# andvg3/LipVQ-VAE

Measured on AMD Instinct MI355X. Metric: actions tokenized/sec (encode+quantize) at B=4096 T=128 K=1024, 1/2/4/8 GPU, higher is better.
Workload: dtype f32

## Files before the change

lipvq-vae_amd/_capi.py:

```python
from __future__ import annotations

import ctypes as C
from pathlib import Path

import torch

import os as _os

_LIB_PATH = Path(_os.environ.get("LIPVQ_HIP_LIBRARY") or (Path(__file__).resolve().parent / "_lipvq_hip.so"))

ACT_NONE, ACT_GELU, ACT_SIGMOID, ACT_RELU = 0, 1, 2, 3
DIST_NORM, DIST_SQSUM = 0, 1
ABI_VERSION = 1

_vp, _i, _i64, _sz = C.c_void_p, C.c_int, C.c_int64, C.c_size_t

SIGNATURES = {
    "lipvq_abi_version": (_i, []),
    "lipvq_last_error": (C.c_char_p, []),
    "lipvq_set_option": (_i, [C.c_char_p, C.c_char_p]),
    "lipvq_get_option": (C.c_char_p, [C.c_char_p]),
    "lipvq_lipschitz_scale_f32": (_i, [_vp, _vp, _vp, _vp, _i, _i, _vp]),
    "lipvq_mlp3_packed_floats": (_sz, [_i, _i, _i, _i]),
    "lipvq_mlp3_pack_f32": (_i, [_vp] * 7 + [_i] * 4 + [_vp]),
# ... 115 lines not shown
            "(python -c 'import __graft_entry__ as g; g.build()' or make -C lipvq-vae_amd/csrc). "
            "There is no CPU fallback for the tokenizer path.")
    lib = C.CDLL(str(_LIB_PATH))
    for name, (res, args) in SIGNATURES.items():
        fn = getattr(lib, name)
        fn.restype, fn.argtypes = res, args
    got = lib.lipvq_abi_version()
    if got != ABI_VERSION:
        raise ImportError(f"lipvq ABI version {got} != expected {ABI_VERSION}")
    return lib


lib = _load()


OPTIONS = ("screen_mode", "tok_shape", "tok_ze_rows", "tok_inplace", "tok_defer_ze", "tok_nt_ze")


def set_option(name: str, value=None) -> None:
    v = None if value is None else str(value).encode()
    if lib.lipvq_set_option(name.encode(), v) != 0:
        raise LipvqLibraryError(lib.lipvq_last_error().decode(errors="replace"))


def get_option(name: str):
    v = lib.lipvq_get_option(name.encode())
    return None if v is None else v.decode()


if _os.environ.get("LIPVQ_DEV_KNOBS") == "1":
    for _o in OPTIONS:
# ... 10 lines not shown
```

lipvq-vae_amd/csrc/lipvq_fused.hip:

```cpp
#include <string.h>
#include <atomic>

#include "lipvq_mlp.h"
#include "lipvq_screen.h"
#include "lipvq_fused_lds.h"

#define FUSED_WAVES 8
#define FUSED_THREADS (FUSED_WAVES * 64)

struct Gelu2 {
    lq_v2f x, t, u, s;
    __device__ __forceinline__ void stage0(float a, float b) {
        x = (lq_v2f){a, b};
        t = x * x;
        u = lq_fma2(t, lq_bc2(0.11111111111111111111f), lq_bc2(-1.0f));
        s = lq_fma2(lq_bc2(0.00012666420661844313f), u, lq_bc2(-0.00043783686123788357f));
        s = lq_fma2(s, u, lq_bc2(0.0008924771682359278f));
    }
    __device__ __forceinline__ void stage1() {
        s = lq_fma2(s, u, lq_bc2(-0.002175821689888835f));
        s = lq_fma2(s, u, lq_bc2(0.005515238270163536f));
        s = lq_fma2(s, u, lq_bc2(-0.01217574905604124f));
        s = lq_fma2(s, u, lq_bc2(0.02415713667869568f));
    }
// ... 47 lines not shown
    int A, D, K;
    float gamma;
    int coarse;
    int inplace;
    int defer_ze;
    int nt_ze;
    int ze_ring;
    int keepz;
};

#ifdef LQ_STAMPS
#define LQ_STAMPS_ENTER()                                                                                            \
    const long long st_top = __builtin_amdgcn_s_memtime();                                                           \
    const long long st_top_rt = (long long)__builtin_amdgcn_s_memrealtime()
#define LQ_STAMPS_PROLOGUE_DONE()                                                                                    \
    long long st_acc[8] = {0, 0, 0, 0, 0, 0, 0, 0}, st_prev;                                                         \
    const long long st_begin = __builtin_amdgcn_s_memtime()
#define LQ_STAMPS_BEGIN_BLOCK() st_prev = __builtin_amdgcn_s_memtime()
#define LQ_STAMP(i) do { const long long t_ = __builtin_amdgcn_s_memtime(); st_acc[i] += t_ - st_prev; st_prev = t_; } while (0)
#define LQ_STAMPS_FLUSH(a, lane, wave, WAVES)                                                                        \
    if (lane == 0) {                                                                                                 \
        long long* dbg = LqWorkspace::from_lists(a.amb_list, a.N).stamps() + ((size_t)blockIdx.x * WAVES + wave) * 16;   \
        for (int i = 0; i < 7; ++i) dbg[i] = st_acc[i];                                                              \
        dbg[7] = 0;                                                                                                  \
        dbg[8] = __builtin_amdgcn_s_memtime() - st_begin;                                                            \
        dbg[9] = st_begin;                                                                                           \
        dbg[10] = st_begin - st_top;                                                                                 \
        dbg[11] = (long long)__builtin_amdgcn_s_memrealtime();                                                       \
        dbg[12] = st_top_rt;                                                                                         \
    }
#else
#define LQ_STAMPS_ENTER() do { } while (0)
#define LQ_STAMPS_PROLOGUE_DONE() do { } while (0)
#define LQ_STAMPS_BEGIN_BLOCK() do { } while (0)
#define LQ_STAMP(i) do { } while (0)
#define LQ_STAMPS_FLUSH(a, lane, wave, WAVES) do { } while (0)
#endif

template <int S, bool TRAIN>
__device__ __forceinline__ void tok_store_ze_tile(const TokArgs& a, const int h, const int64_t ze_shift, const int64_t row, const int t,
                                                  const f32x16& acc) {
    float lo8[8], hi8[8];
#pragma unroll
    for (int j = 0; j < 8; ++j) {
        const auto sw = __builtin_amdgcn_permlane32_swap(__float_as_uint(acc[j]), __float_as_uint(acc[8 + j]), false, false);
        lo8[j] = __uint_as_float(sw[0]);
        hi8[j] = __uint_as_float(sw[1]);
    }
    if (row < a.N && 2 * t + h < S) {
        float4* dst = reinterpret_cast<float4*>(a.ze_out + (size_t)(row - ze_shift) * a.D + 32 * t + 16 * h);
// ... 179 lines not shown
    const unsigned char* src = reinterpret_cast<const unsigned char*>(a.w2q) + (size_t)t_ * (G2 * 1024);
    unsigned char* dst = stage0 + (size_t)buf_ * SLAB_STRIDE;
    unsigned lane16 = (unsigned)lane * 16u;
    asm volatile("" : "+v"(lane16));
#pragma unroll
    for (int j = 0; j < G2 * 1024 / 1024 / WAVES; ++j) {
        const int off = (wave + j * WAVES) * 1024;
        const unsigned long long gaddr = (unsigned long long)(uintptr_t)(src + off) + lane16;
        const unsigned ldsaddr = __builtin_amdgcn_readfirstlane((unsigned)(uintptr_t)(dst + off));
        unsigned m0_keep;
        asm volatile("s_mov_b32 %0, m0\n\ts_mov_b32 m0, %2\n\ts_nop 0\n\tglobal_load_lds_dwordx4 %1, off\n\ts_mov_b32 m0, %0"
                     : "=&s"(m0_keep) : "v"(gaddr), "s"(ldsaddr) : "memory");
    }
}

template <int S, bool FAST, bool TRAIN, int WAVES, bool COARSE = false, bool VQ = false, bool KEEPZ = false>
__device__ __forceinline__ void tokenize_body(const TokArgs& a) {
    static_assert(!(FAST && TRAIN), "training uses the parity arithmetic");
    static_assert(!VQ || !FAST, "the ReLU instance: parity arithmetic");
    static_assert(!KEEPZ || (S <= 4 && !FAST && !TRAIN && !COARSE && !VQ), "z_e kept in registers: the narrow parity instances, decided in place");
    constexpr int THREADS = WAVES * 64;
    constexpr int TCF = COARSE ? fused_ring_tc_coarse(S) : fused_ring_tc(S), NBF = fused_ring_nb(S);
    using Lds = FusedLds<S, FAST>;
    static_assert(Lds::template slices_fit<WAVES, COARSE, KEEPZ>(), "the per-wave slices of the stage ring");
    constexpr size_t SLAB_STRIDE = Lds::SLAB_STRIDE;
    constexpr int T0 = Lds::T0, T1 = Lds::T1, T2 = Lds::T2;
    constexpr int S1 = Lds::S1, S2 = Lds::S2;
    constexpr bool STREAM2 = Lds::STREAM2;
    static_assert(!FAST || (S % 2 == 0 && S <= 8), "fast mode: D in {32, 64, 128}");
    extern __shared__ __attribute__((aligned(16))) unsigned char lds[];
    LQ_STAMPS_ENTER();

    const PackedLayout PL = packed_layout(a.A, 32 * T0, 32 * T1, 16 * S);
    const PrepLayout L = prep_layout(a.K, a.D);
    const int S0 = PL.S0;
    const int S0q = (S0 + 3) / 4;
    const int S0h = (a.A + 15) / 16;
    const Lds lay(a.A);
    float* const w_P0 = reinterpret_cast<float*>(lds);
    float* const w_B0 = w_P0 + lay.template n_P0<int>();
    float* const w_P1 = w_B0 + Lds::N_B0;
    float* const w_B1 = w_P1 + Lds::N_P1;
    float* const w_P2 = w_B1 + Lds::N_B1;
    float* const w_B2 = w_P2 + Lds::N_P2;
    float* const w_mu = w_B2 + Lds::N_B2;
    unsigned char* const stage0 = reinterpret_cast<unsigned char*>(w_mu + Lds::N_MU);
    unsigned* const hist = reinterpret_cast<unsigned*>(stage0 + Lds::template hist_in_ring<COARSE>());
    constexpr size_t STAGES_BYTES = Lds::template stages_bytes<COARSE>(), WSLICE = Lds::template wslice<WAVES, COARSE>();
    const bool use_hist = a.usage && Lds::hist_fits(a.A, a.K);

    const int tid = threadIdx.x, lane = tid & 63;
    const int wave = __builtin_amdgcn_readfirstlane(tid >> 6);
    const int ln = lane & 31, h = lane >> 5;

    const unsigned* hdr = reinterpret_cast<const unsigned*>(a.prep);
    const unsigned char* tiles = a.prep + (COARSE ? L.o_tiles_hi : L.o_tiles);
    const size_t tile_bytes = COARSE ? L.tile_bytes_hi : L.tile_bytes;
    const int sz = lq_scale_exp(1.0f + __uint_as_float(hdr[4]));
    const float fz = lq_pow2f(sz);
    const float fown = lq_pow2f(sz + (int)hdr[3]);
    const float tiny2 = (float)(16 * S) * lq_pow2f(-10 - 2 * sz);
    const int64_t nblk = (a.N + WAVES * 32 - 1) / (WAVES * 32);
    constexpr int XPF = 8;
// ... 156 lines not shown
                }
                if constexpr (KEEPZ) {
                    zkeep[t] = acc;
                } else if (a.ze_out) {
                    if (DEFER_ZE && a.defer_ze && t == T2 - 1) zdef = acc;
                    else store_ze_tile(row, t, acc);
                }
            };

            if constexpr (!FAST) {
                auto bias16 = [&](const float* wb, int t) { return tok_bias16(wb, t, h); };
                f32x16 h0[T0];
                constexpr int NTRIP = (16 * S + 63) / 64;
                constexpr int GP = (STAGES_BYTES >= (size_t)WAVES * 8192) ? 8 : 4;
                constexpr int NROUND = NTRIP * (8 / GP);
                unsigned char* gstage = stage0 + (size_t)wave * WSLICE;
                const bool gnow = DEFER_GATHER && have_pend && a.zq;
                if (gnow) lq_gather_dma<GP>(gstage, a.cb, pend_k, pend_ok, pend_row0, a.N, a.D, lane, 0, 0);
                {
#pragma unroll
                    for (int t = 0; t < T0; ++t) h0[t] = bias16(w_B0, t);
                    if (x_pref) {
#pragma unroll
                        for (int sq = 0; sq < XPF / 4; ++sq) {
                            if (sq < S0q) {
                                float4 av[T0];
#pragma unroll
                                for (int t = 0; t < T0; ++t) av[t] = *reinterpret_cast<const float4*>(w_P0 + ((t * S0q + sq) * 64 + lane_w) * 4);
#pragma unroll
                                for (int q = 0; q < 4; ++q) {
                                    const float bv = tok_x_masked<X_BATCHED, XPF>(x_kmax, 4 * sq + q, xq);
#pragma unroll
                                    for (int t = 0; t < T0; ++t) {
// ... 32 lines not shown
#pragma unroll
                            for (int r = 0; r < 16; ++r) h0[t][r] = pre[r] > 0.0f ? pre[r] : 0.0f;
                        } else if constexpr (LOCKSTEP) {
                            tok_gelu_poly_tile(h0[t], pre);
                            tok_gelu_fixup_lumped(h0[t], pre);
                        } else {
#pragma unroll
                            for (int r = 0; r < 16; r += 2) {
                                const lq_v2f g2 = lq_gelu_poly2((lq_v2f){pre[r], pre[r + 1]});
                                h0[t][r] = g2.x; h0[t][r + 1] = g2.y;
                            }
                            tok_gelu_fixup(h0[t], pre);
                        }
                    }
                }
                if (gnow) {
#pragma unroll
                    for (int rd = 0; rd < NROUND; ++rd) {
                        lq_wait_vmcnt<0>();
                        lq_gather_flush<GP>(gstage, a.zq, pend_ok, pend_row0, a.N, a.D, lane, rd / (8 / GP), GP * (rd % (8 / GP)));
                        if (rd + 1 < NROUND) {
                            asm volatile("s_waitcnt lgkmcnt(0)" ::: "memory");
                            lq_gather_dma<GP>(gstage, a.cb, pend_k, pend_ok, pend_row0, a.N, a.D, lane, (rd + 1) / (8 / GP),
                                              GP * ((rd + 1) % (8 / GP)));
                        }
                    }
                }
                LQ_STAMP(0);
                f32x16 h1[T1];
                f32x16 pend;
                constexpr int G1 = S1 / 4, G2 = S2 / 4;
// ... 140 lines not shown
        for (int r = 0; r < 16; ++r) { m1[r] = INFINITY; m2[r] = INFINITY; k1[r] = 0; }
        LQ_STAMP(3);
        constexpr bool DEFER_X = S <= 4 && !FAST && !TRAIN && !COARSE && !VQ;
        const int64_t blk_next = blk + gridDim.x < nblk ? blk + gridDim.x : blk;
        if (!DEFER_X && x_pref) load_x(blk_next, xq);
        constexpr bool PACKF = S <= 4 || S > 8 || COARSE;
        const float zn = COARSE ? lq_coarse_zn(row_a2, row_n2, row_fz, row_fown, __uint_as_float(hdr[5])) : 0.0f;
        float znr[16];
        if constexpr (COARSE) lq_row_factors(zn, lane, znr);
        else {
#pragma unroll
            for (int r = 0; r < 16; ++r) znr[r] = 0.0f;
        }
        if constexpr (KEEPZ) {
            auto deferred_x = [&]() { load_x(blk_next, xq); };
            lq_screen_core<S, THREADS, TCF, NBF, PACKF, COARSE, 0, decltype(deferred_x), DEFER_X ? XPF : 0>(
                ah, al, tiles, L.ntiles, stage0, tid, frow, znr, m1, m2, k1, false, deferred_x, true, DEFER_X && x_pref);
        } else {
            const bool have_def = DEFER_ZE && a.defer_ze && a.ze_out != nullptr;
            const bool wave_def = __builtin_amdgcn_ballot_w64(row < a.N) != 0ull;
            auto deferred_ze = [&]() {
                if (have_def) store_ze_tile(row, T2 - 1, zdef);
                if (DEFER_X && x_pref) load_x(blk_next, xq);
            };
            lq_screen_core<S, THREADS, TCF, NBF, PACKF, COARSE, 4, decltype(deferred_ze), DEFER_X ? XPF : 0>(
                ah, al, tiles, L.ntiles, stage0, tid, frow, znr, m1, m2, k1, have_def, deferred_ze, wave_def, DEFER_X && x_pref);
        }
        LQ_STAMP(4);
        const unsigned keep_mask = PACKF ? ~((1u << lq_pack_bits(L.ntiles)) - 1u) : 0xffffffffu;
        unsigned char* scratch = stage0 + (size_t)wave * WSLICE;
        int my_k;
        LqDecision dec;
        bool certified = lq_screen_decide<PACKF, COARSE>(m1, m2, k1, scratch, hdr, row_n2, row_fown, a.gamma, a.K, a.D, lane,
                                                         my_k, dec, PACKF ? lq_pow2f(lq_pack_bits(L.ntiles) - 23) : 0.0f, keep_mask,
                                                         zn, tiles, tile_bytes, ScreenCfg<S, TCF, COARSE>::FRAG_BYTES);
        const bool row_sane = VQ || row_n2 >= tiny2;
        certified = certified && row_sane;
        if constexpr (KEEPZ)
            certified = lq_screen_decide_inplace<PACKF, 2 * S, LIPVQ_DIST_NORM, T2>(
                dec, certified, row_sane, my_k, row0, row < a.N, a.amb_count, nullptr, a.cb, a.K, lane, keep_mask, scratch, zkeep);
        else if (!COARSE && a.inplace)
            certified = lq_screen_decide_inplace<PACKF, 2 * S, VQ ? LIPVQ_DIST_SQSUM : LIPVQ_DIST_NORM>(
                dec, certified, row_sane, my_k, row0 - ze_shift, row < a.N, a.amb_count, a.ze_out, a.cb, a.K, lane, keep_mask, scratch);
        else
            lq_screen_emit<PACKF>(dec, certified, row_sane, my_k, row, row < a.N, a.amb_count, a.amb_list, a.N, a.K, lane, keep_mask, scratch);
// ... 10 lines not shown
    }
    if (DEFER_GATHER && have_pend && a.zq) lq_screen_gather(a.cb, a.zq, pend_k, pend_ok, pend_row0, a.N, a.D, lane);
    LQ_STAMPS_FLUSH(a, lane, wave, WAVES);
    lq_ws_publish(a.amb_count);
    if (use_hist) {
        for (int i = tid; i < a.K; i += THREADS) {
            const unsigned c = hist[i];
            if (c) atomicAdd(&a.usage[i], (unsigned long long)c);
        }
    }
}

template <int S, bool FAST, bool TRAIN = false, bool COARSE = false, bool VQ = false, bool KEEPZ = false>
__global__ __launch_bounds__(FUSED_THREADS) void tokenize_kernel(TokArgs a) {
    tokenize_body<S, FAST, TRAIN, FUSED_WAVES, COARSE, VQ, KEEPZ>(a);
}
template <int S, bool FAST, bool TRAIN, bool COARSE = false, bool KEEPZ = false>
__global__ __launch_bounds__(256) __attribute__((amdgpu_waves_per_eu(1, 1))) void tokenize_kernel_w4(TokArgs a) {
    tokenize_body<S, FAST, TRAIN, 4, COARSE, false, KEEPZ>(a);
}

__global__ void mlp3_pack_f16_kernel(const float* __restrict__ W0, const float* __restrict__ W1, const float* __restrict__ W2,
                                     _Float16* __restrict__ out, int A, int J0, int J1, int D) {
    const int S0h = (A + 15) / 16, S1h = J0 / 16, S2h = J1 / 16;
    const int T0 = J0 / 32, T1 = J1 / 32, T2 = (D + 31) / 32;
    const size_t n0 = (size_t)T0 * S0h * 512, n1 = (size_t)T1 * S1h * 512, n2 = (size_t)T2 * S2h * 512;
    size_t g = (size_t)blockIdx.x * blockDim.x + threadIdx.x;
    if (g >= n0 + n1 + n2) return;
    const float* W;
    int K, J, Sh;
// ... 49 lines not shown
    if (hipGetDevice(&dev) == hipSuccess && dev >= 0 && dev < 64) {
        const int t = g_tuned[dev].load(std::memory_order_relaxed);
        if (t) { sc.defer_ze = (t - 1) & 1; sc.nt_ze = ((t - 1) >> 1) & 1; }
    }
    if (const char* e = lq_knob("tok_defer_ze")) sc.defer_ze = e[0] != '0';
    if (const char* e = lq_knob("tok_nt_ze")) sc.nt_ze = e[0] != '0';
    return sc;
}

static int lq_inplace(bool have_ze, int coarse, int K) {
    const char* e = lq_knob("tok_inplace");
    return (have_ze && !coarse && K <= LQ_LISTS_ALL_K && !(e && e[0] == '0')) ? 1 : 0;
}
static int lq_ze_ring(bool caller_wants_ze, int inplace) { return (!caller_wants_ze && inplace) ? 1 : 0; }
static int lq_keepz(int ring, bool parity, int D) { return (ring && parity && lq_screen_S(D) <= 4) ? 1 : 0; }

static int tok_waves(int64_t N) {
    const char* e = lq_knob("tok_shape");
    if (e && !strcmp(e, "w8rg1")) return 8;
    if (e && !strcmp(e, "w4rg1")) return 4;
    return N <= 4 * 32 * 256 ? 4 : 8;
}

__global__ void w2q_pack_kernel(const float* __restrict__ P2, float* __restrict__ out, int T2, int S2) {
    const size_t i = (size_t)blockIdx.x * blockDim.x + threadIdx.x;
    if (i >= (size_t)T2 * (S2 / 4) * 256) return;
    const int q = (int)(i & 3), l = (int)((i >> 2) & 63), sq = (int)((i >> 8) % (S2 / 4)), t = (int)((i >> 8) / (S2 / 4));
    out[i] = P2[((size_t)t * S2 + 4 * sq + q) * 64 + l];
}

template <int S, bool FAST, bool TRAIN, int WAVES, bool COARSE, bool VQ, bool KEEPZ = false>
static int launch_tokenize_as(const TokArgs& a, hipStream_t st) {
    static_assert(WAVES == 8 || !VQ, "the plain VQVAE's instances have 8 waves");
    static LqLdsReserve reserved;
    const size_t lds = fused_lds_bytes<S, FAST>(a.A, a.K);
    if (lds > FUSED_LDS_MAX) return fail(LIPVQ_EUNSUPPORTED, "tokenize: %zu B of LDS needed", lds);
    void (*kfn)(TokArgs);
    if constexpr (WAVES == 4) kfn = tokenize_kernel_w4<S, FAST, TRAIN, COARSE, KEEPZ>;
    else kfn = tokenize_kernel<S, FAST, TRAIN, COARSE, VQ, KEEPZ>;
    if (int rc = lipvq_reserve_lds(reserved, (const void*)kfn, lds, "tokenize")) return rc;
    if (a.w2q) {
        const PackedLayout PL = packed_layout(a.A, 64, 128, a.D);
        const size_t n = LqWorkspace::w2q_floats(a.D);
        hipLaunchKernelGGL(w2q_pack_kernel, dim3((unsigned)((n + 255) / 256)), dim3(256), 0, st, a.packed + PL.oP2,
                           LqWorkspace::from_lists(a.amb_list, a.N).w2q(), PL.T2, PL.S2);
    }
    const int64_t unit = (int64_t)WAVES * 32;
    const int64_t nblk = (a.N + unit - 1) / unit;
    const int64_t cap = 256;
    hipLaunchKernelGGL(kfn, dim3((unsigned)(nblk < cap ? nblk : cap)), dim3(WAVES * 64), lds, st, a);
    return check_launch("tokenize");
}

enum { TOK_TRAIN, TOK_FAST, TOK_PARITY, TOK_VQ };
template <int S, int MODE>
static int launch_tokenize(const TokArgs& a, hipStream_t st) {
    if constexpr (MODE == TOK_TRAIN) {
        return a.coarse ? launch_tokenize_as<S, false, true, 8, true, false>(a, st) : launch_tokenize_as<S, false, true, 8, false, false>(a, st);
    } else if constexpr (MODE == TOK_FAST) {
        if constexpr (S <= 8) return launch_tokenize_as<S, true, false, 8, false, false>(a, st);
        else return LIPVQ_EUNSUPPORTED;
    } else if constexpr (MODE == TOK_PARITY) {
        const int waves = tok_waves(a.N);
        if constexpr (S >= 8) {
            if (a.coarse && waves == 4) return launch_tokenize_as<S, false, false, 4, true, false>(a, st);
        }
        if (a.coarse) return launch_tokenize_as<S, false, false, 8, true, false>(a, st);
        if constexpr (S <= 4) {
            if (a.keepz) return waves == 4 ? launch_tokenize_as<S, false, false, 4, false, false, true>(a, st)
                                           : launch_tokenize_as<S, false, false, 8, false, false, true>(a, st);
        }
        if (waves == 4) return launch_tokenize_as<S, false, false, 4, false, false>(a, st);
        return launch_tokenize_as<S, false, false, 8, false, false>(a, st);
    } else {
        if (a.pre0) return a.coarse ? launch_tokenize_as<S, false, true, 8, true, true>(a, st) : launch_tokenize_as<S, false, true, 8, false, true>(a, st);
        return a.coarse ? launch_tokenize_as<S, false, false, 8, true, true>(a, st) : launch_tokenize_as<S, false, false, 8, false, true>(a, st);
    }
}

extern "C" int lipvq_tokenize_workspace_init(void* workspace, void* stream) {
    if (!workspace) return fail(LIPVQ_EINVAL, "tokenize_workspace_init: null pointer");
    hipError_t e = hipMemsetAsync(workspace, 0, LqWorkspace::kHeaderBytes, (hipStream_t)stream);
// ... 179 lines not shown
```

lipvq-vae_amd/csrc/lipvq_fused_lds.h:

```cpp
#pragma once
#include "lipvq_screen.h"

#define FUSED_HIST_MAX 2048
#define FUSED_LDS_MAX ((size_t)160 * 1024)
#define LQ_RING8_TC 1
#define LQ_RING8_NB 3
#define LQ_RING13_NB 3
constexpr int fused_ring_tc(int S) { return (S <= 2) ? 4 : (S <= 4) ? 2 : (S == 8) ? LQ_RING8_TC : 1; }
constexpr int fused_ring_nb(int S) { return (S <= 4) ? 4 : (S == 8) ? LQ_RING8_NB : LQ_RING13_NB; }
#define LQ_COARSE_TC_WIDE 2
constexpr int fused_ring_tc_coarse(int S) { return S == 8 ? LQ_COARSE_TC_WIDE * fused_ring_tc(S) : fused_ring_tc(S); }

template <int S, bool FAST>
struct FusedLds {
    static constexpr int T0 = 2, T1 = 4, T2 = (S + 1) / 2;
    static constexpr int S1 = 16 * T0, S2 = 16 * T1;
    static constexpr bool STREAM2 = !FAST && S >= LQ_STREAM2_MIN_S;

    static constexpr size_t RING_FINE = lq_ring_bytes<S, fused_ring_tc(S), fused_ring_nb(S)>();
    static constexpr size_t RING_COARSE = (size_t)fused_ring_nb(S) * ScreenCfg<S, fused_ring_tc_coarse(S), true>::STAGE_BYTES + 1024;
    static constexpr size_t RING_BYTES = ((RING_FINE > RING_COARSE ? RING_FINE : RING_COARSE) + 63) & ~(size_t)63;
    template <bool COARSE>
    static constexpr size_t stages_bytes() { return COARSE && RING_COARSE > RING_FINE ? RING_COARSE : RING_FINE; }
    static constexpr size_t SLAB_STRIDE = ScreenCfg<S, fused_ring_tc(S), false>::STAGE_BYTES;
    static constexpr int SLAB_BYTES = (S2 / 4) * 1024;
    static_assert(!STREAM2 || (SLAB_BYTES <= SLAB_STRIDE && 3 * SLAB_STRIDE <= RING_FINE), "slabs ride in the stage ring");
    template <int WAVES, bool COARSE>
    static constexpr size_t wslice() { return (stages_bytes<COARSE>() >= (size_t)WAVES * 8192) ? 8192 : LQ_DECIDE_BYTES; }
    template <int WAVES, bool COARSE, bool KEEPZ>
    static constexpr bool slices_fit() {
        static_assert(stages_bytes<COARSE>() >= (size_t)WAVES * LQ_DECIDE_BYTES, "the decision's per-wave transposes live in the stage ring");
        static_assert(LQ_DECIDE_BYTES >= 4096 && wslice<WAVES, COARSE>() >= LQ_DECIDE_BYTES, "a slice holds the transposes and four staged KiB");
        static_assert(!KEEPZ || wslice<WAVES, COARSE>() >= LQ_DECIDE_BYTES + 64 * S, "KEEPZ: one z_e row behind the decision scratch");
        static_assert(!STREAM2 || SLAB_BYTES % (1024 * WAVES) == 0, "slabs ride in the stage ring");
        return true;
    }

    int k0;
    static constexpr int N_B0 = 32 * T0, N_P1 = FAST ? T1 * (2 * T0) * 256 : T1 * (S1 / 4) * 256;
    static constexpr int N_B1 = 32 * T1, N_P2 = FAST ? T2 * (2 * T1) * 256 : STREAM2 ? 0 : T2 * (S2 / 4) * 256;
    static constexpr int N_B2 = 32 * T2, N_MU = 16 * S;
    __host__ __device__ explicit FusedLds(int A) : k0(FAST ? (A + 15) / 16 : ((A + 1) / 2 + 3) / 4) {}
    template <typename I>
    __host__ __device__ I n_P0() const { return (I)T0 * k0 * 256; }
    template <bool COARSE>
    static constexpr size_t hist_in_ring() { return (stages_bytes<COARSE>() + 63) & ~(size_t)63; }
    __host__ __device__ size_t bytes_nohist() const {
        return (n_P0<size_t>() + N_B0 + N_P1 + N_B1 + N_P2 + N_B2 + N_MU) * sizeof(float) + RING_BYTES;
    }
    __host__ __device__ static bool hist_fits(int A, int K) {
        return K <= FUSED_HIST_MAX && FusedLds(A).bytes_nohist() + (size_t)K * 4 <= FUSED_LDS_MAX;
    }
    __host__ __device__ static size_t bytes(int A, int K) { return FusedLds(A).bytes_nohist() + (hist_fits(A, K) ? (size_t)K * 4 : 0); }
};
```

lipvq-vae_amd/csrc/lipvq_misc.hip:

```cpp
#include <stdlib.h>

#include "lipvq_common.h"

#undef fail
#undef check_launch
static thread_local char g_err[512] = "";

int lipvq_fail(int code, const char* fmt, ...) {
    va_list ap;
    va_start(ap, fmt);
    vsnprintf(g_err, sizeof(g_err), fmt, ap);
    va_end(ap);
    return code;
}

int lipvq_check_launch(const char* what) {
    hipError_t e = hipGetLastError();
    if (e != hipSuccess) return lipvq_fail(LIPVQ_EHIP, "%s: %s", what, hipGetErrorString(e));
    return LIPVQ_OK;
}

static const char* const g_opt_names[] = {"screen_mode", "tok_shape", "tok_ze_rows", "tok_inplace", "tok_defer_ze", "tok_nt_ze"};
constexpr int kNumOpts = (int)(sizeof(g_opt_names) / sizeof(g_opt_names[0]));
static char g_opt_vals[kNumOpts][32];
static bool g_opt_set[kNumOpts];

static int opt_index(const char* name) {
    if (!name) return -1;
    if (!strncmp(name, "LIPVQ_", 6)) name += 6;
    for (int i = 0; i < kNumOpts; ++i) {
        const char* a = g_opt_names[i];
        const char* b = name;
        while (*a && *b && (*a == *b || *a == (*b | 0x20))) { ++a; ++b; }
        if (!*a && !*b) return i;
    }
    return -1;
}
// ... 185 lines not shown
```

lipvq-vae_amd/csrc/lipvq_screen.h:

```cpp
#ifndef LIPVQ_SCREEN_H_
#define LIPVQ_SCREEN_H_
#include <hip/hip_fp16.h>

#include <type_traits>

#include "lipvq_common.h"

typedef _Float16 f16x8 __attribute__((ext_vector_type(8)));

#define LIPVQ_SCREEN_GAMMA 3.814697265625e-06f
#define SCREEN_WAVES 8

struct PrepLayout {
    int S, Dpad, Kpad, ntiles;
    size_t o_hdr, o_mu, o_tiles, tile_bytes, total;
    size_t o_tiles_hi, tile_bytes_hi;
};

#define LIPVQ_SCREEN_GAMMA_WIDE 1.52587890625e-05f
#define LQ_SCREEN_NARROW_MAX_S 13

__host__ __device__ static inline int lq_screen_S(int D) {
    const int s = (D + 15) / 16;
    return D <= 0 ? 0 : s <= 2 ? 2 : s <= 4 ? 4 : s <= 8 ? 8 : s <= 13 ? 13 : s <= 16 ? 16 : s <= 24 ? 24 : s <= 32 ? 32 : 0;
// ... 112 lines not shown
template <int S, int TC_, int NB>
constexpr size_t lq_ring_bytes() { return (size_t)NB * ScreenCfg<S, TC_>::STAGE_BYTES + 1024; }

__host__ __device__ static inline int lq_pack_bits(int ntiles) { int b = 1; while ((1 << b) < ntiles) ++b; return b; }

struct LqNoDeferred { __device__ __forceinline__ void operator()() const {} };
template <int BASE, int NDEF, int NPF>
__device__ __forceinline__ void lq_wait_vmcnt_deferred(bool cd, bool cp) {
    static_assert(BASE + NDEF + NPF < 64, "vmcnt immediate");
    if (NDEF > 0 && NPF > 0 && cd && cp) lq_wait_vmcnt<BASE + NDEF + NPF>();
    else if (NDEF > 0 && cd) lq_wait_vmcnt<BASE + NDEF>();
    else if (NPF > 0 && cp) lq_wait_vmcnt<BASE + NPF>();
    else lq_wait_vmcnt<BASE>();
}
template <int S, int NT, int TC_ = screen_default_tc(S), int NB = 4, bool PACK = false, bool COARSE = false, int NDEF = 0,
          typename DEFERRED = LqNoDeferred, int NPF = 0>
__device__ __forceinline__ void lq_screen_core(const f16x8 (&ah)[S], const f16x8 (&al)[S],
                                               const unsigned char* __restrict__ tiles, int ntiles,
                                               unsigned char* stage0, int tid, const float (&frow)[16], const float (&znr)[16],
                                               float (&m1)[16], float (&m2)[16], int (&k1)[16],
                                               bool have_def = false, DEFERRED deferred = DEFERRED(), bool wave_def = true,
                                               bool have_pf = false) {
    using C = ScreenCfg<S, TC_, COARSE>;
    static_assert(NB >= 3 && NB <= 4, "ring of 3 or 4 stage buffers");
    constexpr int NW = NT / 64;
    constexpr int CHUNKS = (C::STAGE_BYTES + 1023) / 1024;
    constexpr int CPW = (CHUNKS + NW - 1) / NW;
    constexpr int PD = NB - 1;
    constexpr int NSTEP = C::TC * S;
    constexpr int MID = (C::TC >= 2) ? (C::TC / 2) * S : S / 2;
    constexpr int FR = 2;
    constexpr int FD = FR - 1;
    constexpr bool BOOK2 = PACK && !COARSE && S <= 4;
    constexpr bool RING_STATIC = BOOK2 && (8 / C::TC) % NB == 0;
    constexpr int PERIOD = ((C::TC & 1) || (NSTEP % FR)) ? 2 : 1;
    static_assert(C::STAGE_BYTES >= 1024 && C::STAGE_BYTES % 16 == 0, "stage copies are whole KiB pieces");
    static_assert(NSTEP - FD >= MID, "next-stage fragments are read after the hand-over");
    static_assert(CPW * PD < 64, "vmcnt immediate");
    const int lane = tid & 63, ln = lane & 31;
    const int wave = __builtin_amdgcn_readfirstlane(tid >> 6);
    const int nstage = __builtin_amdgcn_readfirstlane(ntiles / C::TC);
    unsigned char* dummy = stage0 + (size_t)NB * C::STAGE_BYTES;
    typedef __attribute__((address_space(3))) void* lds_ptr_t;
    typedef const __attribute__((address_space(1))) void* glb_ptr_t;
    int poff[CPW];
#pragma unroll
    for (int j = 0; j < CPW; ++j) {
        int chunk = wave + j * NW;
        chunk = chunk < CHUNKS ? chunk : CHUNKS - 1;
        const int off = chunk * 1024;
        poff[j] = off + 1024 <= C::STAGE_BYTES ? off : C::STAGE_BYTES - 1024;
    }
    const unsigned lane16 = (unsigned)lane * 16u;
    auto stage_dma = [&](int past, size_t src_off, int rp) {
        const int real = __builtin_amdgcn_readfirstlane(past >> 31);
        const size_t real64 = ((size_t)(unsigned)real << 32) | (unsigned)real;
        const unsigned char* src = tiles + (src_off & real64);
        unsigned char* dbase = dummy - ((NB - rp) * C::STAGE_BYTES & real);
#pragma unroll
        for (int j = 0; j < CPW; ++j) {
            unsigned char* d = dbase + (poff[j] & real);
            __builtin_amdgcn_global_load_lds((glb_ptr_t)(src + poff[j] + lane16), (lds_ptr_t)d, 16, 0, 0);
        }
    };
    typedef const __attribute__((address_space(3))) float* lds_cfloat_t;
    typedef const __attribute__((address_space(3))) f16x8* lds_cfrag_t;
    unsigned norm_lane = (unsigned)(uintptr_t)(lds_ptr_t)(stage0 + C::FRAG_BYTES + ln * 4);
    unsigned frag_lane = (unsigned)(uintptr_t)(lds_ptr_t)(stage0 + lane * 16);
    if constexpr (RING_STATIC) asm volatile("" : "+v"(norm_lane), "+v"(frag_lane));
    auto norm_at = [&](const unsigned char* tb, int extra) {
        return *(lds_cfloat_t)(uintptr_t)(norm_lane + (unsigned)(tb - stage0) + (unsigned)extra);
    };
    auto frag = [&](const unsigned char* tb, int s, int hl) {
        const int piece = COARSE ? s : s * 2 + hl;
        return *(lds_cfrag_t)(uintptr_t)(frag_lane + (unsigned)(tb - stage0) + (unsigned)piece * 1024u);
    };
    lq_wg_barrier();
#pragma unroll
    for (int p = 0; p < PD; ++p) stage_dma(p - nstage, (size_t)p * C::STAGE_BYTES, p);
    static_assert((PD - 1) * CPW + NDEF + NPF < 64, "vmcnt immediate");
    const bool count_def = NDEF > 0 && have_def && wave_def;
    const bool count_pf = NPF > 0 && have_pf;
    if ((NDEF > 0 && have_def) || count_pf) deferred();
    lq_wait_vmcnt_deferred<(PD - 1) * CPW, NDEF, NPF>(count_def, count_pf);
    lq_wg_barrier();

    f32x16 accA, accB;
#pragma unroll
    for (int r = 0; r < 16; ++r) accB[r] = INFINITY;
    float e2A = 0.0f, e2B = 0.0f;
    int codeA = 0, codeB = 0;
    const unsigned keep_mask = PACK ? ~((1u << lq_pack_bits(ntiles)) - 1u) : 0xffffffffu;
    f16x8 fh[FR], fl[FR];
    float e2q[2] = {0.0f, 0.0f};
    float enq[2] = {0.0f, 0.0f};
    float enA = 0.0f, enB = 0.0f;
#pragma unroll
    for (int g = 0; g < FD; ++g) {
        fh[g] = frag(stage0, g, 0);
        if constexpr (!COARSE) fl[g] = frag(stage0, g, 1);
// ... 3 lines not shown
    static_assert(FD <= S, "prologue reads stay in tile 0");
    int buf = 0;
    int past = PD - nstage;
    size_t src_off = (size_t)PD * C::STAGE_BYTES;
    auto do_stage = [&](auto POS, auto RP, auto FIRST, int st) {
        constexpr int par = (decltype(POS)::value * C::TC) & 1;
        constexpr int so = (decltype(POS)::value * NSTEP) % FR;
        const int rp = RP;
        const unsigned char* sb = stage0 + (size_t)rp * C::STAGE_BYTES;
        int nrp = rp + 1; nrp = nrp == NB ? 0 : nrp;
        const unsigned char* nsb = stage0 + (size_t)nrp * C::STAGE_BYTES;
#pragma unroll
        for (int g = 0; g < NSTEP; ++g) {
            const int c = g / S, s = g % S;
            if (g == MID) {
                if ((count_def || count_pf) && FIRST) lq_wait_vmcnt_deferred<(PD >= 2 ? (PD - 2) * CPW : 0), (PD >= 2 ? NDEF : 0), (PD >= 2 ? NPF : 0)>(count_def, count_pf);
                else lq_wait_vmcnt<(PD >= 2 ? (PD - 2) * CPW : 0)>();
                lq_wg_barrier();
                int b = rp + PD; b = b >= NB ? b - NB : b;
                stage_dma(past, src_off, b);
                past += 1;
                src_off += C::STAGE_BYTES;
            }
            f32x16& acc = (((c + par) & 1) == 0) ? accA : accB;
            const f32x16& prev = (((c + par) & 1) == 0) ? accB : accA;
            const float e2_prev = (((c + par) & 1) == 0) ? e2B : e2A;
            const float en_prev = (((c + par) & 1) == 0) ? enB : enA;
            const int code_prev = (((c + par) & 1) == 0) ? codeB : codeA;
            if (s == 0) {
                const float e2c = e2q[(c + par) & 1];
                const float enc = enq[(c + par) & 1];
#pragma unroll
                for (int r = 0; r < 16; ++r) acc[r] = COARSE ? lq_fma(-znr[r], enc, e2c * frow[r]) : 0.0f;
                int code = PACK ? (st * C::TC + c) : (st * C::TC + c) * 32 + ln;
                if constexpr (PACK) asm volatile("" : "+v"(code));
                if (((c + par) & 1) == 0) { e2A = e2c; enA = enc; codeA = code; } else { e2B = e2c; enB = enc; codeB = code; }
            }
// ... 18 lines not shown
            read_ahead();
            __builtin_amdgcn_sched_barrier(0);
            if constexpr (!BOOK2) lq_track_after_mfma<COARSE ? S : 3 * S, PACK, COARSE>(COARSE ? s : 3 * s + 0, prev, e2_prev, en_prev, frow, znr, code_prev, keep_mask, m1, m2, k1);
            __builtin_amdgcn_sched_barrier(0);
            if constexpr (!COARSE) {
                constexpr int NG = BOOK2 ? 2 * S : 3 * S;
                acc = __builtin_amdgcn_mfma_f32_32x32x16_f16(al[s], bh, acc, 0, 0, 0);
                lq_track_after_mfma<NG, PACK>(BOOK2 ? 2 * s + 0 : 3 * s + 1, prev, e2_prev, en_prev, frow, znr, code_prev, keep_mask, m1, m2, k1);
                __builtin_amdgcn_sched_barrier(0);
                acc = __builtin_amdgcn_mfma_f32_32x32x16_f16(ah[s], bl, acc, 0, 0, 0);
                lq_track_after_mfma<NG, PACK>(BOOK2 ? 2 * s + 1 : 3 * s + 2, prev, e2_prev, en_prev, frow, znr, code_prev, keep_mask, m1, m2, k1);
                __builtin_amdgcn_sched_barrier(0);
            }
        }
    };
    if constexpr (RING_STATIC) {
        static_assert(NB == 4 && NB % PERIOD == 0, "one trip = one pass of the ring");
        auto ring_pass = [&](auto FIRST, int st) {
            do_stage(std::integral_constant<int, 0>{}, std::integral_constant<int, 0>{}, FIRST, st);
            do_stage(std::integral_constant<int, 1 % PERIOD>{}, std::integral_constant<int, 1>{}, std::false_type{}, st + 1);
            do_stage(std::integral_constant<int, 2 % PERIOD>{}, std::integral_constant<int, 2>{}, std::false_type{}, st + 2);
            do_stage(std::integral_constant<int, 3 % PERIOD>{}, std::integral_constant<int, 3>{}, std::false_type{}, st + 3);
        };
        ring_pass(std::true_type{}, 0);
        for (int st = NB; st < nstage; st += NB) ring_pass(std::false_type{}, st);
    } else {
        for (int st = 0; st < nstage; st += PERIOD) {
            do_stage(std::integral_constant<int, 0>{}, buf, st == 0, st);
            buf = buf + 1 == NB ? 0 : buf + 1;
            if constexpr (PERIOD == 2) {
                do_stage(std::integral_constant<int, 1>{}, buf, false, st + 1);
// ... 381 lines not shown
            __builtin_amdgcn_wave_barrier();
            bk = lq_lists_row<DCH, DIST>([&](int f) { return zrow[f]; }, cb, K, parts + r * 16, lane, true);
            __builtin_amdgcn_wave_barrier();
        } else {
            const float* zr = z + (size_t)(row0 + r) * D;
            bk = lq_lists_row<DCH, DIST>([&](int f) { return __hip_atomic_load(zr + f, __ATOMIC_RELAXED, __HIP_MEMORY_SCOPE_AGENT); },
                                         cb, K, parts + r * 16, lane, true);
        }
        if (ln == r) { my_k = bk; certified = true; }
    }
    __builtin_amdgcn_wave_barrier();
    return certified;
}

struct LqGatherTrip { float4 val[8]; };
__device__ __forceinline__ void lq_gather_load(LqGatherTrip& g, const float* __restrict__ cb, int my_k, bool row_ok, int64_t row0,
                                               int64_t N, int D, int lane, int trip) {
    const int nvec = D / 4;
    const int v = 16 * trip + (lane & 15);
    const int vc = v < nvec ? v : nvec - 1;
#pragma unroll
    for (int p = 0; p < 8; ++p) {
        const int src_lane = 4 * p + (lane >> 4);
        const int kk = __shfl(my_k, src_lane, 64);
        const bool ok = (__shfl((int)row_ok, src_lane, 64) != 0) && (row0 + src_lane < N);
        g.val[p] = reinterpret_cast<const float4*>(cb + (size_t)(ok ? kk : 0) * D)[vc];
    }
}
__device__ __forceinline__ void lq_gather_store(const LqGatherTrip& g, float* __restrict__ zq, bool row_ok, int64_t row0, int64_t N,
                                                int D, int lane, int trip) {
    const int nvec = D / 4;
    const int v = 16 * trip + (lane & 15);
#pragma unroll
    for (int p = 0; p < 8; ++p) {
        const int src_lane = 4 * p + (lane >> 4);
        const bool ok = (__shfl((int)row_ok, src_lane, 64) != 0) && (row0 + src_lane < N) && (v < nvec);
        if (ok) reinterpret_cast<float4*>(zq + (size_t)(row0 + src_lane) * D)[v] = g.val[p];
    }
}
template <int NP>
__device__ __forceinline__ void lq_gather_dma(unsigned char* wave_stage, const float* __restrict__ cb, int my_k, bool row_ok,
                                              int64_t row0, int64_t N, int D, int lane, int trip, int p0) {
    typedef __attribute__((address_space(3))) void* lds_ptr_t;
    typedef const __attribute__((address_space(1))) void* glb_ptr_t;
    const int nvec = D / 4;
    const int v = 16 * trip + (lane & 15);
    const int vc = v < nvec ? v : nvec - 1;
#pragma unroll
    for (int p = 0; p < NP; ++p) {
        const int src_lane = 4 * (p0 + p) + (lane >> 4);
        const int kk = __shfl(my_k, src_lane, 64);
        const bool ok = (__shfl((int)row_ok, src_lane, 64) != 0) && (row0 + src_lane < N);
// ... 51 lines not shown
```

Baseline: 1.427 billion.

## Keep codebook screening ring continuous across row blocks in the S=4 keepz kernel

Adds a continuous-ring variant of the tokenize kernel for the S=4 keep-z_e instance. The codebook tile DMA ring is no longer drained and re-primed per row block: the prologue barrier and DMA run only on the first block, and the last stages prefetch the next block's first tiles by wrapping src_off to zero. Per-wave scratch slices move behind the ring positions that stay live. The deferred z_q gather is split into half LDS-staged DMA and half register loads with non-temporal stores. It is on by default when LDS fits, and it adds risk around the vmcnt accounting and LDS aliasing between blocks.

```diff
diff --git a/lipvq-vae_amd/_capi.py b/lipvq-vae_amd/_capi.py
--- a/lipvq-vae_amd/_capi.py
+++ b/lipvq-vae_amd/_capi.py
@@ -153,7 +153,7 @@
 lib = _load()
 
 
-OPTIONS = ("screen_mode", "tok_shape", "tok_ze_rows", "tok_inplace", "tok_defer_ze", "tok_nt_ze")
+OPTIONS = ("screen_mode", "tok_shape", "tok_ze_rows", "tok_inplace", "tok_defer_ze", "tok_nt_ze", "tok_ring")
 
 
 def set_option(name: str, value=None) -> None:
diff --git a/lipvq-vae_amd/csrc/lipvq_fused.hip b/lipvq-vae_amd/csrc/lipvq_fused.hip
--- a/lipvq-vae_amd/csrc/lipvq_fused.hip
+++ b/lipvq-vae_amd/csrc/lipvq_fused.hip
@@ -85,10 +85,11 @@
     const long long st_top = __builtin_amdgcn_s_memtime();                                                           \
     const long long st_top_rt = (long long)__builtin_amdgcn_s_memrealtime()
 #define LQ_STAMPS_PROLOGUE_DONE()                                                                                    \
-    long long st_acc[8] = {0, 0, 0, 0, 0, 0, 0, 0}, st_prev;                                                         \
+    long long st_acc[8] = {0, 0, 0, 0, 0, 0, 0, 0}, st_prev, st_open = 0, st_pro = 0;                                \
     const long long st_begin = __builtin_amdgcn_s_memtime()
 #define LQ_STAMPS_BEGIN_BLOCK() st_prev = __builtin_amdgcn_s_memtime()
 #define LQ_STAMP(i) do { const long long t_ = __builtin_amdgcn_s_memtime(); st_acc[i] += t_ - st_prev; st_prev = t_; } while (0)
+#define LQ_STAMPS_SCREEN_ARGS , &st_open, &st_pro
 #define LQ_STAMPS_FLUSH(a, lane, wave, WAVES)                                                                        \
     if (lane == 0) {                                                                                                 \
         long long* dbg = LqWorkspace::from_lists(a.amb_list, a.N).stamps() + ((size_t)blockIdx.x * WAVES + wave) * 16;   \
@@ -99,12 +100,15 @@
         dbg[10] = st_begin - st_top;                                                                                 \
         dbg[11] = (long long)__builtin_amdgcn_s_memrealtime();                                                       \
         dbg[12] = st_top_rt;                                                                                         \
+        dbg[13] = st_open;                                                                                           \
+        dbg[14] = st_pro;                                                                                            \
     }
 #else
 #define LQ_STAMPS_ENTER() do { } while (0)
 #define LQ_STAMPS_PROLOGUE_DONE() do { } while (0)
 #define LQ_STAMPS_BEGIN_BLOCK() do { } while (0)
 #define LQ_STAMP(i) do { } while (0)
+#define LQ_STAMPS_SCREEN_ARGS
 #define LQ_STAMPS_FLUSH(a, lane, wave, WAVES) do { } while (0)
 #endif
 
@@ -314,11 +318,12 @@
     }
 }
 
-template <int S, bool FAST, bool TRAIN, int WAVES, bool COARSE = false, bool VQ = false, bool KEEPZ = false>
+template <int S, bool FAST, bool TRAIN, int WAVES, bool COARSE = false, bool VQ = false, bool KEEPZ = false, bool CONT = false>
 __device__ __forceinline__ void tokenize_body(const TokArgs& a) {
     static_assert(!(FAST && TRAIN), "training uses the parity arithmetic");
     static_assert(!VQ || !FAST, "the ReLU instance: parity arithmetic");
     static_assert(!KEEPZ || (S <= 4 && !FAST && !TRAIN && !COARSE && !VQ), "z_e kept in registers: the narrow parity instances, decided in place");
+    static_assert(!CONT || (KEEPZ && S == 4 && WAVES == 8), "the continuous ring: the metric's instance");
     constexpr int THREADS = WAVES * 64;
     constexpr int TCF = COARSE ? fused_ring_tc_coarse(S) : fused_ring_tc(S), NBF = fused_ring_nb(S);
     using Lds = FusedLds<S, FAST>;
@@ -345,8 +350,10 @@
     float* const w_B2 = w_P2 + Lds::N_P2;
     float* const w_mu = w_B2 + Lds::N_B2;
     unsigned char* const stage0 = reinterpret_cast<unsigned char*>(w_mu + Lds::N_MU);
-    unsigned* const hist = reinterpret_cast<unsigned*>(stage0 + Lds::template hist_in_ring<COARSE>());
-    constexpr size_t STAGES_BYTES = Lds::template stages_bytes<COARSE>(), WSLICE = Lds::template wslice<WAVES, COARSE>();
+    if constexpr (CONT) static_assert(Lds::template cont_slices_fit<WAVES>(), "the per-wave slices behind the ring positions that stay live");
+    unsigned* const hist = reinterpret_cast<unsigned*>(stage0 + (CONT ? Lds::template cont_stages_bytes<WAVES>() : Lds::template hist_in_ring<COARSE>()));
+    constexpr size_t STAGES_BYTES = Lds::template stages_bytes<COARSE>(), WSLICE = CONT ? Lds::CONT_SLICE : Lds::template wslice<WAVES, COARSE>();
+    constexpr size_t SLICE0 = CONT ? Lds::CONT_SLICE0 : 0;
     const bool use_hist = a.usage && Lds::hist_fits(a.A, a.K);
 
     const int tid = threadIdx.x, lane = tid & 63;
@@ -533,9 +540,16 @@
                 constexpr int NTRIP = (16 * S + 63) / 64;
                 constexpr int GP = (STAGES_BYTES >= (size_t)WAVES * 8192) ? 8 : 4;
                 constexpr int NROUND = NTRIP * (8 / GP);
-                unsigned char* gstage = stage0 + (size_t)wave * WSLICE;
+                unsigned char* gstage = stage0 + SLICE0 + (size_t)wave * WSLICE;
                 const bool gnow = DEFER_GATHER && have_pend && a.zq;
-                if (gnow) lq_gather_dma<GP>(gstage, a.cb, pend_k, pend_ok, pend_row0, a.N, a.D, lane, 0, 0);
+                LqGatherTrip gtrip;
+                static_assert(!CONT || (NTRIP == 1 && WSLICE >= 4096), "half a trip of staging, half a trip of registers");
+                if constexpr (CONT) {
+                    if (gnow) {
+                        lq_gather_dma<4>(gstage, a.cb, pend_k, pend_ok, pend_row0, a.N, a.D, lane, 0, 0);
+                        lq_gather_load<4, 4>(gtrip, a.cb, pend_k, pend_ok, pend_row0, a.N, a.D, lane, 0);
+                    }
+                } else if (gnow) lq_gather_dma<GP>(gstage, a.cb, pend_k, pend_ok, pend_row0, a.N, a.D, lane, 0, 0);
                 {
 #pragma unroll
                     for (int t = 0; t < T0; ++t) h0[t] = bias16(w_B0, t);
@@ -598,7 +612,13 @@
                         }
                     }
                 }
-                if (gnow) {
+                if constexpr (CONT) {
+                    if (gnow) {
+                        lq_wait_vmcnt<0>();
+                        lq_gather_flush<4>(gstage, a.zq, pend_ok, pend_row0, a.N, a.D, lane, 0, 0);
+                        lq_gather_store<4, 4, true>(gtrip, a.zq, pend_ok, pend_row0, a.N, a.D, lane, 0);
+                    }
+                } else if (gnow) {
 #pragma unroll
                     for (int rd = 0; rd < NROUND; ++rd) {
                         lq_wait_vmcnt<0>();
@@ -769,8 +789,9 @@
         }
         if constexpr (KEEPZ) {
             auto deferred_x = [&]() { load_x(blk_next, xq); };
-            lq_screen_core<S, THREADS, TCF, NBF, PACKF, COARSE, 0, decltype(deferred_x), DEFER_X ? XPF : 0>(
-                ah, al, tiles, L.ntiles, stage0, tid, frow, znr, m1, m2, k1, false, deferred_x, true, DEFER_X && x_pref);
+            lq_screen_core<S, THREADS, TCF, NBF, PACKF, COARSE, 0, decltype(deferred_x), DEFER_X ? XPF : 0, CONT>(
+                ah, al, tiles, L.ntiles, stage0, tid, frow, znr, m1, m2, k1, false, deferred_x, true, DEFER_X && x_pref,
+                blk == (int64_t)blockIdx.x LQ_STAMPS_SCREEN_ARGS);
         } else {
             const bool have_def = DEFER_ZE && a.defer_ze && a.ze_out != nullptr;
             const bool wave_def = __builtin_amdgcn_ballot_w64(row < a.N) != 0ull;
@@ -783,7 +804,7 @@
         }
         LQ_STAMP(4);
         const unsigned keep_mask = PACKF ? ~((1u << lq_pack_bits(L.ntiles)) - 1u) : 0xffffffffu;
-        unsigned char* scratch = stage0 + (size_t)wave * WSLICE;
+        unsigned char* scratch = stage0 + SLICE0 + (size_t)wave * WSLICE;
         int my_k;
         LqDecision dec;
         bool certified = lq_screen_decide<PACKF, COARSE>(m1, m2, k1, scratch, hdr, row_n2, row_fown, a.gamma, a.K, a.D, lane,
@@ -824,6 +845,10 @@
 template <int S, bool FAST, bool TRAIN = false, bool COARSE = false, bool VQ = false, bool KEEPZ = false>
 __global__ __launch_bounds__(FUSED_THREADS) void tokenize_kernel(TokArgs a) {
     tokenize_body<S, FAST, TRAIN, FUSED_WAVES, COARSE, VQ, KEEPZ>(a);
+}
+template <int S>
+__global__ __launch_bounds__(FUSED_THREADS) void tokenize_kernel_ring(TokArgs a) {
+    tokenize_body<S, false, false, FUSED_WAVES, false, false, true, true>(a);
 }
 template <int S, bool FAST, bool TRAIN, bool COARSE = false, bool KEEPZ = false>
 __global__ __launch_bounds__(256) __attribute__((amdgpu_waves_per_eu(1, 1))) void tokenize_kernel_w4(TokArgs a) {
@@ -903,6 +928,11 @@
 }
 static int lq_ze_ring(bool caller_wants_ze, int inplace) { return (!caller_wants_ze && inplace) ? 1 : 0; }
 static int lq_keepz(int ring, bool parity, int D) { return (ring && parity && lq_screen_S(D) <= 4) ? 1 : 0; }
+template <int S>
+static int lq_tok_ring(int A, int K) {
+    const char* e = lq_knob("tok_ring");
+    return (!(e && e[0] == '0') && FusedLds<S, false>::template cont_fits<FUSED_WAVES>(A, K)) ? 1 : 0;
+}
 
 static int tok_waves(int64_t N) {
     const char* e = lq_knob("tok_shape");
@@ -918,14 +948,17 @@
     out[i] = P2[((size_t)t * S2 + 4 * sq + q) * 64 + l];
 }
 
-template <int S, bool FAST, bool TRAIN, int WAVES, bool COARSE, bool VQ, bool KEEPZ = false>
+template <int S, bool FAST, bool TRAIN, int WAVES, bool COARSE, bool VQ, bool KEEPZ = false, bool CONT = false>
 static int launch_tokenize_as(const TokArgs& a, hipStream_t st) {
     static_assert(WAVES == 8 || !VQ, "the plain VQVAE's instances have 8 waves");
+    static_assert(!CONT || (WAVES == 8 && KEEPZ && !FAST && !TRAIN && !COARSE && !VQ), "the continuous ring's one instance");
     static LqLdsReserve reserved;
-    const size_t lds = fused_lds_bytes<S, FAST>(a.A, a.K);
+    size_t lds = fused_lds_bytes<S, FAST>(a.A, a.K);
+    if constexpr (CONT) lds = FusedLds<S, FAST>::template cont_bytes<WAVES>(a.A, a.K);
     if (lds > FUSED_LDS_MAX) return fail(LIPVQ_EUNSUPPORTED, "tokenize: %zu B of LDS needed", lds);
     void (*kfn)(TokArgs);
-    if constexpr (WAVES == 4) kfn = tokenize_kernel_w4<S, FAST, TRAIN, COARSE, KEEPZ>;
+    if constexpr (CONT) kfn = tokenize_kernel_ring<S>;
+    else if constexpr (WAVES == 4) kfn = tokenize_kernel_w4<S, FAST, TRAIN, COARSE, KEEPZ>;
     else kfn = tokenize_kernel<S, FAST, TRAIN, COARSE, VQ, KEEPZ>;
     if (int rc = lipvq_reserve_lds(reserved, (const void*)kfn, lds, "tokenize")) return rc;
     if (a.w2q) {
@@ -955,6 +988,9 @@
             if (a.coarse && waves == 4) return launch_tokenize_as<S, false, false, 4, true, false>(a, st);
         }
         if (a.coarse) return launch_tokenize_as<S, false, false, 8, true, false>(a, st);
+        if constexpr (S == 4) {
+            if (a.keepz && waves == 8 && lq_tok_ring<S>(a.A, a.K)) return launch_tokenize_as<S, false, false, 8, false, false, true, true>(a, st);
+        }
         if constexpr (S <= 4) {
             if (a.keepz) return waves == 4 ? launch_tokenize_as<S, false, false, 4, false, false, true>(a, st)
                                            : launch_tokenize_as<S, false, false, 8, false, false, true>(a, st);
diff --git a/lipvq-vae_amd/csrc/lipvq_fused_lds.h b/lipvq-vae_amd/csrc/lipvq_fused_lds.h
--- a/lipvq-vae_amd/csrc/lipvq_fused_lds.h
+++ b/lipvq-vae_amd/csrc/lipvq_fused_lds.h
@@ -36,6 +36,26 @@
         return true;
     }
 
+    static constexpr bool CONT_OK = !FAST && S == 4;
+    static constexpr int CONT_KEEP = fused_ring_nb(S) - 1;
+    static constexpr size_t CONT_STAGE = ScreenCfg<S, fused_ring_tc(S), false>::STAGE_BYTES;
+    static constexpr size_t CONT_SLICE0 = (size_t)CONT_KEEP * CONT_STAGE;
+    static constexpr size_t CONT_SLICE = LQ_DECIDE_BYTES + 64 * S;
+    template <int WAVES>
+    static constexpr size_t cont_stages_bytes() {
+        constexpr size_t ring = (size_t)fused_ring_nb(S) * CONT_STAGE, sl = CONT_SLICE0 + (size_t)WAVES * CONT_SLICE;
+        return ((ring > sl ? ring : sl) + 63) & ~(size_t)63;
+    }
+    template <int WAVES>
+    static constexpr bool cont_slices_fit() {
+        static_assert(CONT_OK, "the continuous ring: the parity instance of S = 4");
+        static_assert(CONT_SLICE0 % 16 == 0 && CONT_SLICE % 16 == 0, "16-byte aligned slices (float4 reads of the transposes)");
+        static_assert(CONT_SLICE >= LQ_DECIDE_BYTES + 64 * S, "a slice holds the transposes and one z_e row");
+        static_assert(CONT_SLICE0 >= (size_t)CONT_KEEP * CONT_STAGE, "no slice touches the positions that hold the next block's stages");
+        static_assert(cont_stages_bytes<WAVES>() >= CONT_SLICE0 + (size_t)WAVES * CONT_SLICE, "every wave's slice lies in front of the histogram");
+        return true;
+    }
+
     int k0;
     static constexpr int N_B0 = 32 * T0, N_P1 = FAST ? T1 * (2 * T0) * 256 : T1 * (S1 / 4) * 256;
     static constexpr int N_B1 = 32 * T1, N_P2 = FAST ? T2 * (2 * T1) * 256 : STREAM2 ? 0 : T2 * (S2 / 4) * 256;
@@ -52,4 +72,12 @@
         return K <= FUSED_HIST_MAX && FusedLds(A).bytes_nohist() + (size_t)K * 4 <= FUSED_LDS_MAX;
     }
     __host__ __device__ static size_t bytes(int A, int K) { return FusedLds(A).bytes_nohist() + (hist_fits(A, K) ? (size_t)K * 4 : 0); }
+    template <int WAVES>
+    __host__ __device__ static size_t cont_bytes(int A, int K) {
+        return FusedLds(A).bytes_nohist() - RING_BYTES + cont_stages_bytes<WAVES>() + (size_t)K * 4;
+    }
+    template <int WAVES>
+    __host__ __device__ static bool cont_fits(int A, int K) {
+        return CONT_OK && K <= FUSED_HIST_MAX && cont_bytes<WAVES>(A, K) <= FUSED_LDS_MAX;
+    }
 };
diff --git a/lipvq-vae_amd/csrc/lipvq_misc.hip b/lipvq-vae_amd/csrc/lipvq_misc.hip
--- a/lipvq-vae_amd/csrc/lipvq_misc.hip
+++ b/lipvq-vae_amd/csrc/lipvq_misc.hip
@@ -20,7 +20,7 @@
     return LIPVQ_OK;
 }
 
-static const char* const g_opt_names[] = {"screen_mode", "tok_shape", "tok_ze_rows", "tok_inplace", "tok_defer_ze", "tok_nt_ze"};
+static const char* const g_opt_names[] = {"screen_mode", "tok_shape", "tok_ze_rows", "tok_inplace", "tok_defer_ze", "tok_nt_ze", "tok_ring"};
 constexpr int kNumOpts = (int)(sizeof(g_opt_names) / sizeof(g_opt_names[0]));
 static char g_opt_vals[kNumOpts][32];
 static bool g_opt_set[kNumOpts];
diff --git a/lipvq-vae_amd/csrc/lipvq_screen.h b/lipvq-vae_amd/csrc/lipvq_screen.h
--- a/lipvq-vae_amd/csrc/lipvq_screen.h
+++ b/lipvq-vae_amd/csrc/lipvq_screen.h
@@ -150,13 +150,17 @@
     else lq_wait_vmcnt<BASE>();
 }
 template <int S, int NT, int TC_ = screen_default_tc(S), int NB = 4, bool PACK = false, bool COARSE = false, int NDEF = 0,
-          typename DEFERRED = LqNoDeferred, int NPF = 0>
+          typename DEFERRED = LqNoDeferred, int NPF = 0, bool CONT = false>
 __device__ __forceinline__ void lq_screen_core(const f16x8 (&ah)[S], const f16x8 (&al)[S],
                                                const unsigned char* __restrict__ tiles, int ntiles,
                                                unsigned char* stage0, int tid, const float (&frow)[16], const float (&znr)[16],
                                                float (&m1)[16], float (&m2)[16], int (&k1)[16],
                                                bool have_def = false, DEFERRED deferred = DEFERRED(), bool wave_def = true,
-                                               bool have_pf = false) {
+                                               bool have_pf = false, bool first_block = true
+#ifdef LQ_STAMPS
+                                               , long long* st_open = nullptr, long long* st_pro = nullptr
+#endif
+                                               ) {
     using C = ScreenCfg<S, TC_, COARSE>;
     static_assert(NB >= 3 && NB <= 4, "ring of 3 or 4 stage buffers");
     constexpr int NW = NT / 64;
@@ -173,6 +177,7 @@
     static_assert(C::STAGE_BYTES >= 1024 && C::STAGE_BYTES % 16 == 0, "stage copies are whole KiB pieces");
     static_assert(NSTEP - FD >= MID, "next-stage fragments are read after the hand-over");
     static_assert(CPW * PD < 64, "vmcnt immediate");
+    static_assert(!CONT || (RING_STATIC && PD == 3 && NDEF == 0), "the continuous ring: whole passes of a four-buffer ring, no deferred stores");
     const int lane = tid & 63, ln = lane & 31;
     const int wave = __builtin_amdgcn_readfirstlane(tid >> 6);
     const int nstage = __builtin_amdgcn_readfirstlane(ntiles / C::TC);
@@ -189,6 +194,14 @@
     }
     const unsigned lane16 = (unsigned)lane * 16u;
     auto stage_dma = [&](int past, size_t src_off, int rp) {
+        if constexpr (CONT) {
+            const unsigned char* src = tiles + src_off;
+            unsigned char* dbase = stage0 + (size_t)rp * C::STAGE_BYTES;
+#pragma unroll
+            for (int j = 0; j < CPW; ++j)
+                __builtin_amdgcn_global_load_lds((glb_ptr_t)(src + poff[j] + lane16), (lds_ptr_t)(dbase + poff[j]), 16, 0, 0);
+            return;
+        }
         const int real = __builtin_amdgcn_readfirstlane(past >> 31);
         const size_t real64 = ((size_t)(unsigned)real << 32) | (unsigned)real;
         const unsigned char* src = tiles + (src_off & real64);
@@ -211,15 +224,29 @@
         const int piece = COARSE ? s : s * 2 + hl;
         return *(lds_cfrag_t)(uintptr_t)(frag_lane + (unsigned)(tb - stage0) + (unsigned)piece * 1024u);
     };
-    lq_wg_barrier();
-#pragma unroll
-    for (int p = 0; p < PD; ++p) stage_dma(p - nstage, (size_t)p * C::STAGE_BYTES, p);
+#ifdef LQ_STAMPS
+    const long long st_t0 = __builtin_amdgcn_s_memtime();
+#endif
+    const bool prologue = !CONT || first_block;
+    if (prologue) {
+        lq_wg_barrier();
+#ifdef LQ_STAMPS
+        if (st_open) *st_open += __builtin_amdgcn_s_memtime() - st_t0;
+#endif
+#pragma unroll
+        for (int p = 0; p < PD; ++p) stage_dma(p - nstage, (size_t)p * C::STAGE_BYTES, p);
+    }
     static_assert((PD - 1) * CPW + NDEF + NPF < 64, "vmcnt immediate");
     const bool count_def = NDEF > 0 && have_def && wave_def;
     const bool count_pf = NPF > 0 && have_pf;
     if ((NDEF > 0 && have_def) || count_pf) deferred();
-    lq_wait_vmcnt_deferred<(PD - 1) * CPW, NDEF, NPF>(count_def, count_pf);
-    lq_wg_barrier();
+    if (prologue) {
+        lq_wait_vmcnt_deferred<(PD - 1) * CPW, NDEF, NPF>(count_def, count_pf);
+        lq_wg_barrier();
+    }
+#ifdef LQ_STAMPS
+    if (st_pro) *st_pro += __builtin_amdgcn_s_memtime() - st_t0;
+#endif
 
     f32x16 accA, accB;
 #pragma unroll
@@ -253,13 +280,18 @@
         for (int g = 0; g < NSTEP; ++g) {
             const int c = g / S, s = g % S;
             if (g == MID) {
-                if ((count_def || count_pf) && FIRST) lq_wait_vmcnt_deferred<(PD >= 2 ? (PD - 2) * CPW : 0), (PD >= 2 ? NDEF : 0), (PD >= 2 ? NPF : 0)>(count_def, count_pf);
+                if constexpr (CONT) {
+                    constexpr int first = decltype(FIRST)::value;
+                    if constexpr (first == 1 || first == 2) lq_wait_vmcnt_deferred<CPW, 0, NPF>(false, count_pf);
+                    else lq_wait_vmcnt<CPW>();
+                } else if ((count_def || count_pf) && FIRST) lq_wait_vmcnt_deferred<(PD >= 2 ? (PD - 2) * CPW : 0), (PD >= 2 ? NDEF : 0), (PD >= 2 ? NPF : 0)>(count_def, count_pf);
                 else lq_wait_vmcnt<(PD >= 2 ? (PD - 2) * CPW : 0)>();
                 lq_wg_barrier();
                 int b = rp + PD; b = b >= NB ? b - NB : b;
                 stage_dma(past, src_off, b);
                 past += 1;
                 src_off += C::STAGE_BYTES;
+                if constexpr (CONT) src_off = past == 0 ? 0 : src_off;
             }
             f32x16& acc = (((c + par) & 1) == 0) ? accA : accB;
             const f32x16& prev = (((c + par) & 1) == 0) ? accB : accA;
@@ -308,7 +340,17 @@
             }
         }
     };
-    if constexpr (RING_STATIC) {
+    if constexpr (CONT) {
+        auto ring_pass = [&](auto PEEL, int st) {
+            constexpr int pl = decltype(PEEL)::value;
+            do_stage(std::integral_constant<int, 0>{}, std::integral_constant<int, 0>{}, std::integral_constant<int, pl * 1>{}, st);
+            do_stage(std::integral_constant<int, 1 % PERIOD>{}, std::integral_constant<int, 1>{}, std::integral_constant<int, pl * 2>{}, st + 1);
+            do_stage(std::integral_constant<int, 2 % PERIOD>{}, std::integral_constant<int, 2>{}, std::integral_constant<int, 0>{}, st + 2);
+            do_stage(std::integral_constant<int, 3 % PERIOD>{}, std::integral_constant<int, 3>{}, std::integral_constant<int, 0>{}, st + 3);
+        };
+        ring_pass(std::integral_constant<int, 1>{}, 0);
+        for (int st = NB; st < nstage; st += NB) ring_pass(std::integral_constant<int, 0>{}, st);
+    } else if constexpr (RING_STATIC) {
         static_assert(NB == 4 && NB % PERIOD == 0, "one trip = one pass of the ring");
         auto ring_pass = [&](auto FIRST, int st) {
             do_stage(std::integral_constant<int, 0>{}, std::integral_constant<int, 0>{}, FIRST, st);
@@ -720,28 +762,35 @@
 }
 
 struct LqGatherTrip { float4 val[8]; };
+template <int P0 = 0, int NP = 8>
 __device__ __forceinline__ void lq_gather_load(LqGatherTrip& g, const float* __restrict__ cb, int my_k, bool row_ok, int64_t row0,
                                                int64_t N, int D, int lane, int trip) {
     const int nvec = D / 4;
     const int v = 16 * trip + (lane & 15);
     const int vc = v < nvec ? v : nvec - 1;
 #pragma unroll
-    for (int p = 0; p < 8; ++p) {
+    for (int p = P0; p < P0 + NP; ++p) {
         const int src_lane = 4 * p + (lane >> 4);
         const int kk = __shfl(my_k, src_lane, 64);
         const bool ok = (__shfl((int)row_ok, src_lane, 64) != 0) && (row0 + src_lane < N);
         g.val[p] = reinterpret_cast<const float4*>(cb + (size_t)(ok ? kk : 0) * D)[vc];
     }
 }
+template <int P0 = 0, int NP = 8, bool NT = false>
 __device__ __forceinline__ void lq_gather_store(const LqGatherTrip& g, float* __restrict__ zq, bool row_ok, int64_t row0, int64_t N,
                                                 int D, int lane, int trip) {
     const int nvec = D / 4;
     const int v = 16 * trip + (lane & 15);
 #pragma unroll
-    for (int p = 0; p < 8; ++p) {
+    for (int p = P0; p < P0 + NP; ++p) {
         const int src_lane = 4 * p + (lane >> 4);
         const bool ok = (__shfl((int)row_ok, src_lane, 64) != 0) && (row0 + src_lane < N) && (v < nvec);
-        if (ok) reinterpret_cast<float4*>(zq + (size_t)(row0 + src_lane) * D)[v] = g.val[p];
+        if constexpr (NT) {
+            typedef float lq_f4v __attribute__((ext_vector_type(4)));
+            if (ok) __builtin_nontemporal_store((lq_f4v){g.val[p].x, g.val[p].y, g.val[p].z, g.val[p].w}, reinterpret_cast<lq_f4v*>(zq + (size_t)(row0 + src_lane) * D) + v);
+        } else {
+            if (ok) reinterpret_cast<float4*>(zq + (size_t)(row0 + src_lane) * D)[v] = g.val[p];
+        }
     }
 }
 template <int NP>
```

Result: no change. 1.436 billion, median of 6 (+0.6%).
